# matter-labs/era-zkevm_test_harness

Measured on AMD Instinct MI355X. Metric: base-layer circuits/sec (2^20 rows); full-block synth wall-time 1/8 GPU, higher is better.
Workload: dtype u64 (Goldilocks, p = 2^64 - 2^32 + 1)

## Files before the change

### era_zkevm_test_harness_amd/csrc/gl64.cuh

```cuda
#pragma once
#include <hip/hip_runtime.h>
#include <stdint.h>

namespace gl {

typedef uint64_t u64;
typedef uint32_t u32;

constexpr u64 P = 0xFFFFFFFF00000001ULL;
constexpr u64 EPS = 0xFFFFFFFFULL;

#define GL_HD __host__ __device__ __forceinline__

GL_HD u64 canon(u64 x) { return x >= P ? x - P : x; }

GL_HD u64 add(u64 a, u64 b) {
#if defined(__HIP_DEVICE_COMPILE__)
    unsigned long long s, t;
    const bool c = __builtin_uaddll_overflow(a, b, &s);
    const bool c2 = __builtin_uaddll_overflow(s, c ? EPS : 0, &t);
    return t + (c2 ? EPS : 0);
#else
    u64 s = a + b;
    u64 c = s < a ? EPS : 0;
    u64 t = s + c;
    u64 c2 = t < s ? EPS : 0;
    return t + c2;
#endif
}

GL_HD u64 add_canon(u64 a, u64 c) {
#if defined(__HIP_DEVICE_COMPILE__)
    unsigned long long s;
    const bool w = __builtin_uaddll_overflow(a, c, &s);
    u32 f = w ? 1u : 0u;
    u64 r, dead;
    asm("v_mad_u64_u32 %0, %1, %2, -1, %3" : "=v"(r), "=s"(dead) : "v"(f), "v"((u64)s));
    return r;
#else
    u64 s = a + c;
    return s < a ? s + EPS : s;
#endif
}

GL_HD u64 sub(u64 a, u64 b) {
#if defined(__HIP_DEVICE_COMPILE__)
    unsigned long long d, t;
    const bool br = __builtin_usubll_overflow(a, b, &d);
    const bool br2 = __builtin_usubll_overflow(d, br ? EPS : 0, &t);
    return t - (br2 ? EPS : 0);
#else
    u64 d = a - b;
    u64 br = a < b ? EPS : 0;
    u64 t = d - br;
    u64 br2 = t > d ? EPS : 0;
    return t - br2;
#endif
}

GL_HD u64 neg(u64 a) { return sub(0, a); }

GL_HD u64 reduce128(u64 lo, u64 hi) {
    u64 hh = hi >> 32, hl = hi & EPS;
#if defined(__HIP_DEVICE_COMPILE__)
    unsigned long long t0, r;
    const bool borrow = __builtin_usubll_overflow(lo, hh, &t0);
    t0 -= borrow ? EPS : 0;
    const u64 t1 = (hl << 32) - hl;
    const bool carry = __builtin_uaddll_overflow(t0, t1, &r);
    r += carry ? EPS : 0;
    return r;
#else
    u64 t0 = lo - hh;
    if (lo < hh) t0 -= EPS;
    u64 t1 = hl * EPS;
    u64 r = t0 + t1;
    if (r < t1) r += EPS;
    return r;
#endif
}

#if defined(__HIPCC__)
__device__ __forceinline__ u64 mul_sched(u64 a, u64 b) {
#if !defined(__HIP_DEVICE_COMPILE__)
    return 0;
#else
    const u32 a0 = (u32)a, a1 = (u32)(a >> 32), b0 = (u32)b, b1 = (u32)(b >> 32);
    const u32 zero = 0;
    u64 p, q, h;
    u32 cm;
    asm("v_mad_u64_u32 %0, s[100:101], %4, %6, 0\n\t"
        "v_mad_u64_u32 %1, s[100:101], %4, %7, 0\n\t"
        "v_mad_u64_u32 %2, s[100:101], %5, %7, 0\n\t"
        "v_mad_u64_u32 %1, vcc, %5, %6, %1\n\t"
        "v_addc_co_u32 %3, vcc, 0, %8, vcc"
        : "=&v"(p), "=&v"(q), "=&v"(h), "=&v"(cm)
        : "v"(a0), "v"(a1), "v"(b0), "v"(b1), "v"(zero)
        : "vcc", "s100", "s101");
    const u32 p0 = (u32)p, p1 = (u32)(p >> 32), q0 = (u32)q, q1 = (u32)(q >> 32), h0 = (u32)h, h1 = (u32)(h >> 32);
    u32 r0, r1, w1, g0, g1, m, t0, t1;
    asm("v_add_co_u32 %2, vcc, %8, %10\n\t"
        "v_addc_co_u32 %3, vcc, %12, %11, vcc\n\t"
        "v_addc_co_u32 %4, vcc, %13, %14, vcc\n\t"
        "v_sub_co_u32 %0, vcc, %9, %4\n\t"
        "v_subbrev_co_u32 %1, vcc, 0, %2, vcc\n\t"
        "v_cndmask_b32 %5, 0, -1, vcc\n\t"
        "v_sub_co_u32 %0, vcc, %0, %5\n\t"
        "v_subbrev_co_u32 %1, vcc, 0, %1, vcc\n\t"
        "v_sub_co_u32 %6, vcc, 0, %3\n\t"
        "v_subbrev_co_u32 %7, vcc, 0, %3, vcc\n\t"
        "v_add_co_u32 %0, vcc, %0, %6\n\t"
        "v_addc_co_u32 %1, vcc, %1, %7, vcc\n\t"
        "v_cndmask_b32 %5, 0, -1, vcc\n\t"
        "v_add_co_u32 %0, vcc, %0, %5\n\t"
        "v_addc_co_u32 %1, vcc, 0, %1, vcc"
        : "=&v"(r0), "=&v"(r1), "=&v"(w1), "=&v"(g0), "=&v"(g1), "=&v"(m), "=&v"(t0), "=&v"(t1)
        : "v"(p1), "v"(p0), "v"(q0), "v"(q1), "v"(h0), "v"(h1), "v"(cm)
        : "vcc");
    return ((u64)r1 << 32) | r0;
#endif
}
#endif

#if defined(__HIPCC__)
__device__ __forceinline__ u64 mul_cyc(u64 a, u64 b) {
#if !defined(__HIP_DEVICE_COMPILE__)
    return 0;
#else
    const u32 a0 = (u32)a, a1 = (u32)(a >> 32), b0 = (u32)b, b1 = (u32)(b >> 32);
    u64 p, q, h, x, cm, c1, cw, cw2, bw, b1f, dead;
    asm("v_mad_u64_u32 %0, %1, %2, %3, 0" : "=v"(p), "=s"(dead) : "v"(a0), "v"(b0));
    asm("v_mad_u64_u32 %0, %1, %2, %3, 0" : "=v"(q), "=s"(dead) : "v"(a0), "v"(b1));
    asm("v_mad_u64_u32 %0, %1, %2, %3, 0" : "=v"(h), "=s"(dead) : "v"(a1), "v"(b1));
    asm("v_mad_u64_u32 %0, %1, %2, %3, %4" : "=v"(q), "=s"(cm) : "v"(a1), "v"(b0), "v"(q));
    const u32 p0 = (u32)p, p1 = (u32)(p >> 32), q0 = (u32)q, q1 = (u32)(q >> 32), h0 = (u32)h, h1 = (u32)(h >> 32);
    u32 w1, w2, w3, y0, y1, dlo, dhi;
    asm("v_add_co_u32_e64 %0, %1, %2, %3" : "=v"(w1), "=s"(cw) : "v"(p1), "v"(q0));
    asm("v_addc_co_u32_e64 %0, %1, %2, %3, %4" : "=v"(w2), "=s"(cw2) : "v"(h0), "v"(q1), "s"(cw));
    asm("v_addc_co_u32_e64 %0, %1, %2, 0, %3" : "=v"(w3), "=s"(dead) : "v"(h1), "s"(cw2));
    const u64 lo = ((u64)w1 << 32) | p0;
    asm("v_mad_u64_u32 %0, %1, %2, -1, %3" : "=v"(x), "=s"(c1) : "v"(w2), "v"(lo));
    const u32 x0 = (u32)x, x1 = (u32)(x >> 32);
    asm("v_subb_co_u32_e64 %0, %1, %2, %3, %4" : "=v"(y0), "=s"(bw) : "v"(x0), "v"(w3), "s"(cm));
    asm("v_subbrev_co_u32_e64 %0, %1, 0, %2, %3" : "=v"(y1), "=s"(b1f) : "v"(x1), "s"(bw));
    const u64 mp = c1 & ~b1f, mn = b1f & ~c1;
    asm("v_cndmask_b32_e64 %0, 0, -1, %1" : "=v"(dhi) : "s"(mn));
    asm("v_cndmask_b32_e64 %0, 0, 1, %1" : "=v"(dlo) : "s"(mn));
    asm("v_cndmask_b32_e64 %0, %1, -1, %2" : "=v"(dlo) : "v"(dlo), "s"(mp));
    u64 d = ((u64)dhi << 32) | dlo;
    asm("" : "+v"(d));
    return (((u64)y1 << 32) | y0) + d;
#endif
}
#endif

GL_HD u64 mul_lat(u64 a, u64 b) {
#if defined(__HIP_DEVICE_COMPILE__) && defined(GL_MUL_SCHEDULED_EVERYWHERE)
    return mul_sched(a, b);
#else
#if defined(__HIP_DEVICE_COMPILE__)
    const u32 a0 = (u32)a, a1 = (u32)(a >> 32), b0 = (u32)b, b1 = (u32)(b >> 32);
    const u64 t = (u64)a0 * b0;
    const u64 t1 = (u64)a0 * b1 + (t >> 32);
    const u64 t2 = (u64)a1 * b0 + (u32)t1;
    u64 lo = (t2 << 32) | (u32)t;
    u64 hi = (u64)a1 * b1 + (t1 >> 32) + (t2 >> 32);
#else
    unsigned __int128 w = (unsigned __int128)a * b;
    u64 lo = (u64)w, hi = (u64)(w >> 64);
#endif
    return reduce128(lo, hi);
#endif
}

GL_HD u64 mul(u64 a, u64 b) {
#if defined(__HIP_DEVICE_COMPILE__) && !defined(GL_MUL_COMPILER_FORM)
    return mul_cyc(a, b);
#else
    return mul_lat(a, b);
#endif
}

GL_HD u64 sqr(u64 a) { return mul(a, a); }

GL_HD u64 mul_add(u64 a, u64 b, u64 c) { return add(mul(a, b), c); }

GL_HD u64 pow7(u64 x) {
    u64 x2 = sqr(x);
    u64 x3 = mul(x2, x);
    u64 x4 = sqr(x2);
    return mul(x3, x4);
}
GL_HD u64 pow7_lat(u64 x) {
    u64 x2 = mul_lat(x, x);
    u64 x3 = mul_lat(x2, x);
    u64 x4 = mul_lat(x2, x2);
    return mul_lat(x3, x4);
}

GL_HD u64 mul_pow2(u64 x, u32 s) {
    u64 lo = x << s;
    u64 hi = s ? (x >> (64 - s)) : 0;
    u64 t1 = (hi << 32) - hi;
    u64 r = lo + t1;
    if (r < t1) r += EPS;
    return r;
}

GL_HD u64 mul_small(u64 x, u32 k) {
    u64 l = (x & EPS) * k;
    u64 h = (x >> 32) * k;
    u64 hh = h >> 32, hl = h & EPS;
    u64 r = l + (hl << 32);
    u64 c = r < l ? EPS : 0;
    u64 t = hh * EPS;
    u64 r2 = r + c;
    u64 r3 = r2 + t;
    if (r3 < t) r3 += EPS;
    return r3;
}

GL_HD u64 pow(u64 a, u64 e) {
    u64 r = 1;
    while (e) {
        if (e & 1) r = mul(r, a);
        a = sqr(a);
        e >>= 1;
    }
    return r;
}

GL_HD u64 sqr_n(u64 a, int n) {
    for (int i = 0; i < n; i++) a = sqr(a);
    return a;
}
GL_HD u64 inv(u64 a) {
    const u64 e2 = mul(sqr(a), a);
    const u64 e3 = mul(sqr(e2), a);
    const u64 e6 = mul(sqr_n(e3, 3), e3);
    const u64 e12 = mul(sqr_n(e6, 6), e6);
    const u64 e24 = mul(sqr_n(e12, 12), e12);
    const u64 e30 = mul(sqr_n(e24, 6), e6);
    const u64 e31 = mul(sqr(e30), a);
    const u64 e32 = mul(sqr(e31), a);
    return mul(sqr_n(e31, 33), e32);
}

}
```

### era_zkevm_test_harness_amd/csrc/poseidon2.cuh

```cuda
#pragma once
#include "gl64.cuh"
#include "../../include/zkw_poseidon2_params.h"

namespace p2 {
using gl::u32;
using gl::u64;

static __constant__ u64 c_rc[P2_TOTAL_ROUNDS * P2_WIDTH] = P2_ROUND_CONSTANTS_INIT;
static __constant__ u32 c_shift[P2_WIDTH] = P2_INTERNAL_DIAG_SHIFTS_INIT;

__host__ __device__ __forceinline__ u64 rc_at(int i) {
#if defined(__HIP_DEVICE_COMPILE__)
    return c_rc[i];
#else
    return P2_ROUND_CONSTANTS[i];
#endif
}
__host__ __device__ __forceinline__ u32 shift_at(int i) {
#if defined(__HIP_DEVICE_COMPILE__)
    return c_shift[i];
#else
    return P2_INTERNAL_DIAG_SHIFTS[i];
#endif
}

struct Wide {
    u64 lo;
    u32 hi;
};
GL_HD Wide wide(u64 x) { Wide r; r.lo = x; r.hi = 0; return r; }
GL_HD Wide wadd(Wide a, Wide b) {
    Wide r;
    r.lo = a.lo + b.lo;
    r.hi = a.hi + b.hi + (r.lo < a.lo ? 1u : 0u);
    return r;
}
GL_HD Wide wshl(Wide a, u32 s) {
    Wide r;
    r.lo = a.lo << s;
    r.hi = (a.hi << s) | (u32)(a.lo >> (64 - s));
    return r;
}
GL_HD u64 wreduce(Wide a) {
    u64 t = ((u64)a.hi << 32) - a.hi;
    u64 r = a.lo + t;
    u64 c = r < t ? gl::EPS : 0;
    return r + c;
}

GL_HD void m4w(const u64 x[4], Wide t[4]) {
    Wide t0 = wadd(wide(x[0]), wide(x[1])), t1 = wadd(wide(x[2]), wide(x[3]));
    Wide t2 = wadd(wshl(wide(x[1]), 1), t1), t3 = wadd(wshl(wide(x[3]), 1), t0);
    Wide t4 = wadd(wshl(t1, 2), t3), t5 = wadd(wshl(t0, 2), t2);
    t[0] = wadd(t3, t5); t[1] = t5; t[2] = wadd(t2, t4); t[3] = t4;
}

#if defined(__HIP_DEVICE_COMPILE__)
__device__ __forceinline__ u64 mad_acc(u32 a, u32 k, u64 acc) {
    u64 r, dead;
    asm("v_mad_u64_u32 %0, %1, %2, %3, %4" : "=v"(r), "=s"(dead) : "v"(a), "s"(k), "v"(acc));
    return r;
}
__device__ __forceinline__ u64 mad_acc1(u32 a, u64 acc) {
    u64 r, dead;
    asm("v_mad_u64_u32 %0, %1, %2, 1, %3" : "=v"(r), "=s"(dead) : "v"(a), "v"(acc));
    return r;
}
__device__ __forceinline__ u64 mad_acc2(u32 a, u64 acc) {
    u64 r, dead;
    asm("v_mad_u64_u32 %0, %1, %2, 2, %3" : "=v"(r), "=s"(dead) : "v"(a), "v"(acc));
    return r;
}
__device__ __forceinline__ u64 wp_reduce(u64 L, u64 H) {
    const u32 l0 = (u32)L, l1 = (u32)(L >> 32), h0 = (u32)H, h1 = (u32)(H >> 32);
    u32 n1, k, f;
    u64 c, c2, dead, r;
    asm("v_add_co_u32_e64 %0, %1, %2, %3" : "=v"(n1), "=s"(c) : "v"(l1), "v"(h0));
    asm("v_addc_co_u32_e64 %0, %1, %2, 0, %3" : "=v"(k), "=s"(dead) : "v"(h1), "s"(c));
    const u64 x = ((u64)n1 << 32) | l0;
    asm("v_mad_u64_u32 %0, %1, %2, -1, %3" : "=v"(r), "=s"(c2) : "v"(k), "v"(x));
    asm("v_cndmask_b32_e64 %0, 0, 1, %1" : "=v"(f) : "s"(c2));
    asm("v_mad_u64_u32 %0, %1, %2, -1, %3" : "=v"(r), "=s"(dead) : "v"(f), "v"(r));
    return r;
}
__device__ __forceinline__ void m4_plane(u32 a0, u32 a1, u32 a2, u32 a3, u64 y[4]) {
    const u64 t0 = mad_acc1(a0, (u64)a1), t1 = mad_acc1(a2, (u64)a3);
    const u64 t2 = mad_acc2(a1, t1), t3 = mad_acc2(a3, t0);
    const u64 t4 = (t1 << 2) + t3, t5 = (t0 << 2) + t2;
    y[0] = t3 + t5; y[1] = t5; y[2] = t2 + t4; y[3] = t4;
}
#endif

GL_HD void external(u64 s[12]) {
#if defined(__HIP_DEVICE_COMPILE__) && !defined(P2_LINEAR_WIDE)
    u64 L[12], H[12];
#pragma unroll
    for (int b = 0; b < 3; b++) {
        m4_plane((u32)s[4 * b], (u32)s[4 * b + 1], (u32)s[4 * b + 2], (u32)s[4 * b + 3], L + 4 * b);
        m4_plane((u32)(s[4 * b] >> 32), (u32)(s[4 * b + 1] >> 32), (u32)(s[4 * b + 2] >> 32), (u32)(s[4 * b + 3] >> 32), H + 4 * b);
    }
#pragma unroll
    for (int i = 0; i < 4; i++) {
        const u64 cl = L[i] + L[4 + i] + L[8 + i], ch = H[i] + H[4 + i] + H[8 + i];
#pragma unroll
        for (int b = 0; b < 3; b++) s[4 * b + i] = wp_reduce(L[4 * b + i] + cl, H[4 * b + i] + ch);
    }
#else
    Wide t[12];
    m4w(s, t); m4w(s + 4, t + 4); m4w(s + 8, t + 8);
#pragma unroll
    for (int i = 0; i < 4; i++) {
        Wide col = wadd(wadd(t[i], t[4 + i]), t[8 + i]);
        s[i] = wreduce(wadd(t[i], col)); s[4 + i] = wreduce(wadd(t[4 + i], col)); s[8 + i] = wreduce(wadd(t[8 + i], col));
    }
#endif
}

GL_HD void internal(u64 s[12]) {
    constexpr u32 SH[12] = P2_INTERNAL_DIAG_SHIFTS_INIT;
#if defined(__HIP_DEVICE_COMPILE__) && !defined(P2_LINEAR_WIDE)
    u64 sl = (u64)(u32)s[0], sh = s[0] >> 32;
#pragma unroll
    for (int i = 1; i < 12; i++) { sl = mad_acc1((u32)s[i], sl); sh = mad_acc1((u32)(s[i] >> 32), sh); }
#pragma unroll
    for (int i = 0; i < 12; i++) {
        const u64 l = SH[i] ? mad_acc((u32)s[i], 1u << SH[i], sl) : mad_acc1((u32)s[i], sl);
        const u64 h = SH[i] ? mad_acc((u32)(s[i] >> 32), 1u << SH[i], sh) : mad_acc1((u32)(s[i] >> 32), sh);
        s[i] = wp_reduce(l, h);
    }
#else
    Wide sum = wide(s[0]);
#pragma unroll
    for (int i = 1; i < 12; i++) sum = wadd(sum, wide(s[i]));
#pragma unroll
    for (int i = 0; i < 12; i++) s[i] = wreduce(wadd(SH[i] ? wshl(wide(s[i]), SH[i]) : wide(s[i]), sum));
#endif
}

#ifndef P2_SBOX_GROUP
#define P2_SBOX_GROUP 3
#endif
template <bool LAT = false>
GL_HD void full_round(u64 s[12], int r) {
#pragma unroll
    for (int i = 0; i < 12; i++) {
        s[i] = LAT ? gl::pow7_lat(gl::add_canon(s[i], rc_at(12 * r + i))) : gl::pow7(gl::add_canon(s[i], rc_at(12 * r + i)));
#if defined(__HIP_DEVICE_COMPILE__)
        if (!LAT && (i + 1) % P2_SBOX_GROUP == 0) __builtin_amdgcn_sched_barrier(0);
#endif
    }
    external(s);
}

template <bool LAT = false>
GL_HD void partial_round(u64 s[12], int r) {
    s[0] = LAT ? gl::pow7_lat(gl::add_canon(s[0], rc_at(12 * r))) : gl::pow7(gl::add_canon(s[0], rc_at(12 * r)));
    internal(s);
}

template <bool LAT = false>
GL_HD void permute(u64 s[12]) {
    external(s);
    int r = 0;
    for (int k = 0; k < P2_HALF_FULL_ROUNDS; k++, r++) full_round<LAT>(s, r);
    for (int k = 0; k < P2_PARTIAL_ROUNDS; k++, r++) partial_round<LAT>(s, r);
    for (int k = 0; k < P2_HALF_FULL_ROUNDS; k++, r++) full_round<LAT>(s, r);
}
GL_HD void permute_lat(u64 s[12]) { permute<true>(s); }

#if defined(__HIPCC__)
template <int CTRL>
__device__ __forceinline__ u32 dpp32(u32 v) {
    return (u32)__builtin_amdgcn_update_dpp((int)0, (int)v, CTRL, 0xF, 0xF, false);
}
template <int CTRL>
__device__ __forceinline__ u64 dpp64(u64 v) {
    u32 lo = dpp32<CTRL>((u32)v), hi = dpp32<CTRL>((u32)(v >> 32));
    return ((u64)hi << 32) | lo;
}
constexpr int QP_ROT1 = 1 | (2 << 2) | (3 << 4) | (0 << 6);
constexpr int QP_ROT2 = 2 | (3 << 2) | (0 << 4) | (1 << 6);
constexpr int QP_ROT3 = 3 | (0 << 2) | (1 << 4) | (2 << 6);
constexpr int QP_SWAP1 = 1 | (0 << 2) | (3 << 4) | (2 << 6);
constexpr int QP_BCAST0 = 0;
constexpr int ROW_ROR4 = 0x124, ROW_ROR8 = 0x128, ROW_ROR12 = 0x12C;

template <int CTRL>
__device__ __forceinline__ Wide wdpp(Wide a) {
    Wide r;
    r.lo = dpp64<CTRL>(a.lo);
    r.hi = dpp32<CTRL>(a.hi);
    return r;
}
__device__ __forceinline__ u64 add_rc_sched(u64 x, u64 c) {
    u32 r0, r1, m;
    asm("v_add_co_u32 %0, vcc, %3, %5\n\t"
        "v_addc_co_u32 %1, vcc, %4, %6, vcc\n\t"
        "v_cndmask_b32 %2, 0, -1, vcc\n\t"
        "v_add_co_u32 %0, vcc, %0, %2\n\t"
        "v_addc_co_u32 %1, vcc, 0, %1, vcc"
        : "=&v"(r0), "=&v"(r1), "=&v"(m)
        : "v"((u32)x), "v"((u32)(x >> 32)), "v"((u32)c), "v"((u32)(c >> 32))
        : "vcc");
    return ((u64)r1 << 32) | r0;
}
__device__ __forceinline__ u64 pow7_sched(u64 x) {
    const u64 x2 = gl::mul_sched(x, x), x3 = gl::mul_sched(x2, x), x4 = gl::mul_sched(x2, x2);
    return gl::mul_sched(x3, x4);
}

struct Coop {
    u64 rc_full[2 * P2_HALF_FULL_ROUNDS];
    u32 ka, kb, kd;
    u32 shift;
    u32 rsh, hi_mask;
    bool active;
    bool first;
    bool second;

    __device__ __forceinline__ void init(int g) {
        active = g < 12;
        first = g == 0;
        second = g == 1;
#pragma unroll
        for (int k = 0; k < 2 * P2_HALF_FULL_ROUNDS; k++) {
            int round = k < P2_HALF_FULL_ROUNDS ? k : k + P2_PARTIAL_ROUNDS;
            rc_full[k] = active ? c_rc[12 * round + g] : 0;
        }
        bool even = (g & 1) == 0;
        ka = even ? 5u : 6u;
        kb = even ? 7u : 1u;
        kd = even ? 3u : 4u;
        shift = active ? c_shift[g] : 0;
        rsh = (32u - shift) & 31u;
        hi_mask = shift ? 0xffffffffu : 0u;
    }

    __device__ __forceinline__ u64 external(u64 x) const {
        u64 a = x, b = dpp64<QP_ROT1>(x), c = dpp64<QP_ROT2>(x), d = dpp64<QP_ROT3>(x);
        u64 L = (a & gl::EPS) * ka + (b & gl::EPS) * kb + (c & gl::EPS) + (d & gl::EPS) * kd;
        u64 H = (a >> 32) * ka + (b >> 32) * kb + (c >> 32) + (d >> 32) * kd;
        u32 r0, r1, t0, t1, t2, u0, u1, u2, e0, e1, e2;
        asm volatile(
            "v_add_co_u32 %3, vcc, %11, %13\n\t"
            "v_addc_co_u32 %4, vcc, 0, %14, vcc\n\t"
            "s_nop 0\n\t"
            "v_add_co_u32_dpp %5, vcc, %12, %12 row_ror:8 row_mask:0xf bank_mask:0xf\n\t"
            "v_addc_co_u32_dpp %6, vcc, %3, %3, vcc row_ror:8 row_mask:0xf bank_mask:0xf\n\t"
            "v_addc_co_u32_dpp %7, vcc, %4, %4, vcc row_ror:8 row_mask:0xf bank_mask:0xf\n\t"
            "v_add_co_u32_dpp %5, vcc, %5, %5 row_ror:4 row_mask:0xf bank_mask:0xf\n\t"
            "v_addc_co_u32_dpp %6, vcc, %6, %6, vcc row_ror:4 row_mask:0xf bank_mask:0xf\n\t"
            "v_addc_co_u32_dpp %7, vcc, %7, %7, vcc row_ror:4 row_mask:0xf bank_mask:0xf\n\t"
            "v_add_co_u32 %0, vcc, %12, %5\n\t"
            "v_addc_co_u32 %1, vcc, %3, %6, vcc\n\t"
            "v_addc_co_u32 %2, vcc, %4, %7, vcc\n\t"
            "v_sub_co_u32 %8, vcc, 0, %2\n\t"
            "v_subbrev_co_u32 %9, vcc, 0, %2, vcc\n\t"
            "v_add_co_u32 %0, vcc, %0, %8\n\t"
            "v_addc_co_u32 %1, vcc, %1, %9, vcc\n\t"
            "v_cndmask_b32 %10, 0, -1, vcc\n\t"
            "v_add_co_u32 %0, vcc, %0, %10\n\t"
            "v_addc_co_u32 %1, vcc, 0, %1, vcc"
            : "=&v"(r0), "=&v"(r1), "=&v"(t0), "=&v"(t1), "=&v"(t2), "=&v"(u0), "=&v"(u1), "=&v"(u2), "=&v"(e0), "=&v"(e1), "=&v"(e2)
            : "v"((u32)(L >> 32)), "v"((u32)L), "v"((u32)H), "v"((u32)(H >> 32))
            : "vcc");
        const u64 y = ((u64)r1 << 32) | r0;
        return active ? y : 0;
    }

    __device__ __forceinline__ u64 internal(u64 x) const {
        const u32 x0 = (u32)x, x1 = (u32)(x >> 32);
        u32 s0, s1, s2;
        const u32 zero = 0;
        asm volatile(
            "s_nop 1\n\t"
            "v_add_co_u32_dpp %0, vcc, %3, %3 row_ror:8 row_mask:0xf bank_mask:0xf\n\t"
            "v_addc_co_u32_dpp %1, vcc, %4, %4, vcc row_ror:8 row_mask:0xf bank_mask:0xf\n\t"
            "v_addc_co_u32 %2, vcc, 0, %5, vcc\n\t"
            "v_add_co_u32_dpp %0, vcc, %0, %0 row_ror:4 row_mask:0xf bank_mask:0xf\n\t"
            "v_addc_co_u32_dpp %1, vcc, %1, %1, vcc row_ror:4 row_mask:0xf bank_mask:0xf\n\t"
            "v_addc_co_u32_dpp %2, vcc, %2, %2, vcc row_ror:4 row_mask:0xf bank_mask:0xf\n\t"
            "v_add_co_u32_dpp %0, vcc, %0, %0 quad_perm:[2,3,0,1] row_mask:0xf bank_mask:0xf\n\t"
            "v_addc_co_u32_dpp %1, vcc, %1, %1, vcc quad_perm:[2,3,0,1] row_mask:0xf bank_mask:0xf\n\t"
            "v_addc_co_u32_dpp %2, vcc, %2, %2, vcc quad_perm:[2,3,0,1] row_mask:0xf bank_mask:0xf\n\t"
            "v_add_co_u32_dpp %0, vcc, %0, %0 quad_perm:[1,0,3,2] row_mask:0xf bank_mask:0xf\n\t"
            "v_addc_co_u32_dpp %1, vcc, %1, %1, vcc quad_perm:[1,0,3,2] row_mask:0xf bank_mask:0xf\n\t"
            "v_addc_co_u32_dpp %2, vcc, %2, %2, vcc quad_perm:[1,0,3,2] row_mask:0xf bank_mask:0xf"
            : "=&v"(s0), "=&v"(s1), "=&v"(s2)
            : "v"(x0), "v"(x1), "v"(zero)
            : "vcc");
        const u64 mlo = x << shift;
        const u32 m2 = (x1 >> rsh) & hi_mask;
        u32 r0, r1;
        u32 t0, t1, t2, t3;
        asm volatile(
            "v_add_co_u32 %0, vcc, %6, %9\n\t"
            "v_addc_co_u32 %1, vcc, %7, %10, vcc\n\t"
            "v_addc_co_u32 %2, vcc, %8, %11, vcc\n\t"
            "v_sub_co_u32 %3, vcc, 0, %2\n\t"
            "v_subbrev_co_u32 %4, vcc, 0, %2, vcc\n\t"
            "v_add_co_u32 %0, vcc, %0, %3\n\t"
            "v_addc_co_u32 %1, vcc, %1, %4, vcc\n\t"
            "v_cndmask_b32 %5, 0, -1, vcc\n\t"
            "v_add_co_u32 %0, vcc, %0, %5\n\t"
            "v_addc_co_u32 %1, vcc, 0, %1, vcc"
            : "=&v"(r0), "=&v"(r1), "=&v"(t0), "=&v"(t1), "=&v"(t2), "=&v"(t3)
            : "v"((u32)mlo), "v"((u32)(mlo >> 32)), "v"(m2), "v"(s0), "v"(s1), "v"(s2)
            : "vcc");
        const u64 y = ((u64)r1 << 32) | r0;
        return active ? y : 0;
    }

    __device__ __forceinline__ u64 permute(u64 x) const {
        x = external(x);
#pragma unroll
        for (int k = 0; k < P2_HALF_FULL_ROUNDS; k++) x = external(pow7_sched(add_rc_sched(x, rc_full[k])));
        for (int k = 0; k < P2_PARTIAL_ROUNDS; k++) {
            u64 rc = c_rc[12 * (P2_HALF_FULL_ROUNDS + k)];
            u64 sx = pow7_pair(add_rc_sched(x, rc));
            x = internal(first ? sx : x);
        }
#pragma unroll
        for (int k = 0; k < P2_HALF_FULL_ROUNDS; k++)
            x = external(pow7_sched(add_rc_sched(x, rc_full[P2_HALF_FULL_ROUNDS + k])));
        return x;
    }

    __device__ __forceinline__ u64 pow7_pair(u64 t) const {
        const u64 t0 = dpp64<QP_BCAST0>(t);
        const u64 x2 = gl::mul_sched(t0, t0);
        const u64 b = second ? x2 : t0;
        const u64 y = gl::mul_sched(x2, b);
        return gl::mul_sched(y, dpp64<QP_SWAP1>(y));
    }
};

template <class Put>
__device__ __forceinline__ u64 coop_flattened(const Coop& co, u64 x, u32 g, Put&& put) {
    if (co.active) put(g, gl::canon(x));
    x = co.external(x);
#pragma unroll
    for (int k = 0; k < P2_HALF_FULL_ROUNDS; k++) {
        x = co.external(pow7_sched(add_rc_sched(x, co.rc_full[k])));
        if (co.active) put(12 * (k + 1) + g, gl::canon(x));
    }
    for (int k = 0; k < P2_PARTIAL_ROUNDS; k++) {
        const u64 rc = c_rc[12 * (P2_HALF_FULL_ROUNDS + k)];
        const u64 sx = co.pow7_pair(add_rc_sched(x, rc));
        if (co.first) put(12 * (P2_HALF_FULL_ROUNDS + 1) + k, gl::canon(sx));
        x = co.internal(co.first ? sx : x);
    }
#pragma unroll
    for (int k = 0; k < P2_HALF_FULL_ROUNDS; k++) {
        x = co.external(pow7_sched(add_rc_sched(x, co.rc_full[P2_HALF_FULL_ROUNDS + k])));
        if (co.active) put(12 * (P2_HALF_FULL_ROUNDS + 1) + P2_PARTIAL_ROUNDS + 12 * k + g, gl::canon(x));
    }
    return gl::canon(x);
}


#if defined(P2_Q4_PARTIAL_SCHED)
#define Q4_PARTIAL_MUL gl::mul_sched
#else
#define Q4_PARTIAL_MUL gl::mul_lat
#endif
#if defined(P2_Q4_FULL_CYC)
#define Q4_FULL_POW7 gl::pow7
#else
#define Q4_FULL_POW7 gl::pow7_lat
#endif
template <int CTRL>
__device__ __forceinline__ u32 qdpp32(u32 v) {
    return (u32)__builtin_amdgcn_update_dpp((int)0, (int)v, CTRL, 0xF, 0xF, true);
}
template <int CTRL>
__device__ __forceinline__ u64 qdpp64(u64 v) {
    return ((u64)qdpp32<CTRL>((u32)(v >> 32)) << 32) | qdpp32<CTRL>((u32)v);
}

struct Coop4 {
    u64 rc_full[2 * P2_HALF_FULL_ROUNDS][3];
    u32 ka, kb, kd;
    u32 pw[3];
    bool first;
    bool second;

    __device__ __forceinline__ void init(int j) {
        first = j == 0;
        second = j == 1;
#pragma unroll
        for (int k = 0; k < 2 * P2_HALF_FULL_ROUNDS; k++) {
            int round = k < P2_HALF_FULL_ROUNDS ? k : k + P2_PARTIAL_ROUNDS;
#pragma unroll
            for (int c = 0; c < 3; c++) rc_full[k][c] = c_rc[12 * round + 4 * c + j];
        }
        bool even = (j & 1) == 0;
        ka = even ? 5u : 6u;
        kb = even ? 7u : 1u;
        kd = even ? 3u : 4u;
#pragma unroll
        for (int c = 0; c < 3; c++) pw[c] = 1u << c_shift[4 * c + j];
    }

#if defined(__HIP_DEVICE_COMPILE__)
    static __device__ __forceinline__ u64 mad_v(u32 a, u32 k, u64 acc) {
        u64 r, dead;
        asm("v_mad_u64_u32 %0, %1, %2, %3, %4" : "=v"(r), "=s"(dead) : "v"(a), "v"(k), "v"(acc));
        return r;
    }
    template <bool SC = false>
    static __device__ __forceinline__ u64 add_rc(u64 x, u32 c0, u32 c1);
#endif

    __device__ __forceinline__ u64 m4_plane(u32 a) const {
        const u32 b = qdpp32<QP_ROT1>(a), c = qdpp32<QP_ROT2>(a), d = qdpp32<QP_ROT3>(a);
#if defined(__HIP_DEVICE_COMPILE__)
        return mad_v(d, kd, mad_v(b, kb, mad_v(a, ka, (u64)c)));
#else
        return (u64)a * ka + (u64)b * kb + c + (u64)d * kd;
#endif
    }

    __device__ __forceinline__ void external(u64 x[3]) const {
#if defined(__HIP_DEVICE_COMPILE__)
        u64 L[3], H[3];
#pragma unroll
        for (int c = 0; c < 3; c++) { L[c] = m4_plane((u32)x[c]); H[c] = m4_plane((u32)(x[c] >> 32)); }
        const u64 cl = L[0] + L[1] + L[2], ch = H[0] + H[1] + H[2];
#pragma unroll
        for (int c = 0; c < 3; c++) x[c] = wp_reduce(L[c] + cl, H[c] + ch);
#endif
    }

    __device__ __forceinline__ void internal(u64 x[3]) const {
#if defined(__HIP_DEVICE_COMPILE__)
        const u64 pl = mad_acc1((u32)x[0], mad_acc1((u32)x[1], (u64)(u32)x[2]));
        const u64 ph = mad_acc1((u32)(x[0] >> 32), mad_acc1((u32)(x[1] >> 32), x[2] >> 32));
        u32 l0, l1, h0, h1;
        asm volatile(
            "s_nop 1\n\t"
            "v_add_co_u32_dpp %0, vcc, %4, %4 quad_perm:[2,3,0,1] row_mask:0xf bank_mask:0xf\n\t"
            "v_addc_co_u32_dpp %1, vcc, %5, %5, vcc quad_perm:[2,3,0,1] row_mask:0xf bank_mask:0xf\n\t"
            "v_add_co_u32_dpp %2, vcc, %6, %6 quad_perm:[2,3,0,1] row_mask:0xf bank_mask:0xf\n\t"
            "v_addc_co_u32_dpp %3, vcc, %7, %7, vcc quad_perm:[2,3,0,1] row_mask:0xf bank_mask:0xf\n\t"
            "v_add_co_u32_dpp %0, vcc, %0, %0 quad_perm:[1,0,3,2] row_mask:0xf bank_mask:0xf\n\t"
            "v_addc_co_u32_dpp %1, vcc, %1, %1, vcc quad_perm:[1,0,3,2] row_mask:0xf bank_mask:0xf\n\t"
            "v_add_co_u32_dpp %2, vcc, %2, %2 quad_perm:[1,0,3,2] row_mask:0xf bank_mask:0xf\n\t"
            "v_addc_co_u32_dpp %3, vcc, %3, %3, vcc quad_perm:[1,0,3,2] row_mask:0xf bank_mask:0xf"
            : "=&v"(l0), "=&v"(l1), "=&v"(h0), "=&v"(h1)
            : "v"((u32)pl), "v"((u32)(pl >> 32)), "v"((u32)ph), "v"((u32)(ph >> 32))
            : "vcc");
        const u64 sl = ((u64)l1 << 32) | l0, sh = ((u64)h1 << 32) | h0;
#pragma unroll
        for (int c = 0; c < 3; c++) x[c] = wp_reduce(mad_v((u32)x[c], pw[c], sl), mad_v((u32)(x[c] >> 32), pw[c], sh));
#endif
    }

    __device__ __forceinline__ void permute(u64 x[3]) const {
#if defined(__HIP_DEVICE_COMPILE__)
        constexpr u64 RC[P2_TOTAL_ROUNDS * P2_WIDTH] = P2_ROUND_CONSTANTS_INIT;
        external(x);
#pragma unroll
        for (int k = 0; k < P2_HALF_FULL_ROUNDS; k++) {
#pragma unroll
            for (int c = 0; c < 3; c++) x[c] = Q4_FULL_POW7(add_rc(x[c], (u32)rc_full[k][c], (u32)(rc_full[k][c] >> 32)));
            external(x);
        }
#pragma unroll
        for (int k = 0; k < P2_PARTIAL_ROUNDS; k++) {
            constexpr int R0 = 12 * P2_HALF_FULL_ROUNDS;
            const u64 rc = RC[R0 + 12 * k];
            const u64 t0 = qdpp64<QP_BCAST0>(add_rc<true>(x[0], (u32)rc, (u32)(rc >> 32)));
            const u64 x2 = Q4_PARTIAL_MUL(t0, t0);
            const u64 y = Q4_PARTIAL_MUL(x2, second ? x2 : t0);
            const u64 sx = Q4_PARTIAL_MUL(y, qdpp64<QP_SWAP1>(y));
            x[0] = first ? sx : x[0];
            internal(x);
        }
#pragma unroll
        for (int k = 0; k < P2_HALF_FULL_ROUNDS; k++) {
#pragma unroll
            for (int c = 0; c < 3; c++)
                x[c] = Q4_FULL_POW7(add_rc(x[c], (u32)rc_full[P2_HALF_FULL_ROUNDS + k][c], (u32)(rc_full[P2_HALF_FULL_ROUNDS + k][c] >> 32)));
            external(x);
        }
#endif
    }
};
#if defined(__HIP_DEVICE_COMPILE__)
#define P2_Q4_ADD_RC(C0)                                                             \
    asm("v_add_co_u32 %0, vcc, %3, %5\n\t"                                          \
        "v_addc_co_u32 %1, vcc, %4, %6, vcc\n\t"                                    \
        "v_subb_co_u32 %2, vcc, %0, %0, vcc"           \
        : "=&v"(r0), "=&v"(r1), "=&v"(m)                                              \
        : C0(c0), "v"(c1), "v"((u32)x), "v"((u32)(x >> 32))                           \
        : "vcc")
template <bool SC>
__device__ __forceinline__ u64 Coop4::add_rc(u64 x, u32 c0, u32 c1) {
    u32 r0, r1, m;
    if constexpr (SC) P2_Q4_ADD_RC("s"); else P2_Q4_ADD_RC("v");
    return mad_acc1(m, ((u64)r1 << 32) | r0);
}
#undef P2_Q4_ADD_RC
#endif

struct Coop2 {
    u64 rc_full[2 * P2_HALF_FULL_ROUNDS][6];
    u32 shift[6];
    bool first;

    __device__ __forceinline__ void init(int j) {
        first = j == 0;
#pragma unroll
        for (int k = 0; k < 2 * P2_HALF_FULL_ROUNDS; k++) {
            const int round = k < P2_HALF_FULL_ROUNDS ? k : k + P2_PARTIAL_ROUNDS;
#pragma unroll
            for (int c = 0; c < 3; c++) {
                rc_full[k][2 * c] = c_rc[12 * round + 4 * c + 2 * j];
                rc_full[k][2 * c + 1] = c_rc[12 * round + 4 * c + 2 * j + 1];
            }
        }
#pragma unroll
        for (int c = 0; c < 3; c++) {
            shift[2 * c] = c_shift[4 * c + 2 * j];
            shift[2 * c + 1] = c_shift[4 * c + 2 * j + 1];
        }
    }

    __device__ __forceinline__ void external(u64 x[6]) const {
        Wide A[3], B[3];
#pragma unroll
        for (int c = 0; c < 3; c++) {
            const Wide own = wadd(wide(x[2 * c]), wide(x[2 * c + 1]));
            const Wide oth = wdpp<QP_SWAP1>(own);
            const u64 p1 = dpp64<QP_SWAP1>(x[2 * c + 1]);
            B[c] = wadd(wadd(wshl(own, 2), wshl(wide(x[2 * c + 1]), 1)), oth);
            A[c] = wadd(wadd(B[c], wshl(wide(p1), 1)), own);
        }
        const Wide colA = wadd(wadd(A[0], A[1]), A[2]), colB = wadd(wadd(B[0], B[1]), B[2]);
#pragma unroll
        for (int c = 0; c < 3; c++) {
            x[2 * c] = wreduce(wadd(A[c], colA));
            x[2 * c + 1] = wreduce(wadd(B[c], colB));
        }
    }

    __device__ __forceinline__ void internal(u64 x[6]) const {
        Wide s = wide(x[0]);
#pragma unroll
        for (int i = 1; i < 6; i++) s = wadd(s, wide(x[i]));
        s = wadd(s, wdpp<QP_SWAP1>(s));
#pragma unroll
        for (int i = 0; i < 6; i++) {
            Wide m;
            m.lo = x[i] << shift[i];
            m.hi = (u32)((x[i] >> 1) >> (63 - shift[i]));
            x[i] = wreduce(wadd(m, s));
        }
    }

    __device__ __forceinline__ void permute(u64 x[6]) const {
        external(x);
#pragma unroll
        for (int k = 0; k < P2_HALF_FULL_ROUNDS; k++) {
#pragma unroll
            for (int i = 0; i < 6; i++) x[i] = gl::pow7_lat(gl::add(x[i], rc_full[k][i]));
            external(x);
        }
        for (int k = 0; k < P2_PARTIAL_ROUNDS; k++) {
            const u64 rc = c_rc[12 * (P2_HALF_FULL_ROUNDS + k)];
            const u64 sx = gl::pow7_lat(gl::add(x[0], rc));
            x[0] = first ? sx : x[0];
            internal(x);
        }
#pragma unroll
        for (int k = 0; k < P2_HALF_FULL_ROUNDS; k++) {
#pragma unroll
            for (int i = 0; i < 6; i++) x[i] = gl::pow7_lat(gl::add(x[i], rc_full[P2_HALF_FULL_ROUNDS + k][i]));
            external(x);
        }
    }
};
#endif

}
```

Baseline: 3049.

## Hand-schedule Goldilocks mul/sqr/reduce in asm for Coop4 Poseidon2 rounds

Adds hand-written inline-asm Goldilocks multiply, square (three partial products plus a shift instead of four) and a shared reduction, and uses them for the full-round pow7 and the partial-round S-box in the cooperative 4-lane Poseidon2 permutation. It also rewrites the external and internal linear layers as batched v_mad_u64_u32 sequences with a three-way fused Goldilocks reduction, replacing the per-element mad_v and wp_reduce calls. The goal is fewer VALU instructions and shorter dependency chains in the hash inner loop. In exchange it removes the compile-time selectable multiply variants, and because the asm blocks reuse vcc heavily they may limit compiler scheduling or hide subtle carry bugs.

```diff
diff --git a/era_zkevm_test_harness_amd/csrc/gl64.cuh b/era_zkevm_test_harness_amd/csrc/gl64.cuh
--- a/era_zkevm_test_harness_amd/csrc/gl64.cuh
+++ b/era_zkevm_test_harness_amd/csrc/gl64.cuh
@@ -120,6 +120,69 @@
     return ((u64)r1 << 32) | r0;
 #endif
 }
+
+__device__ __forceinline__ u64 lone_reduce(u64 p, u64 q, u64 h, u32 cm) {
+#if !defined(__HIP_DEVICE_COMPILE__)
+    return 0;
+#else
+    u32 y0, y1, w2, w3, m;
+    asm("v_add_co_u32 %1, vcc, %5, %7\n\t"
+        "v_addc_co_u32 %2, vcc, %9, %8, vcc\n\t"
+        "v_addc_co_u32 %3, vcc, %10, %11, vcc\n\t"
+        "v_sub_co_u32 %0, vcc, %6, %3\n\t"
+        "v_subbrev_co_u32 %1, vcc, 0, %1, vcc\n\t"
+        "v_subb_co_u32 %4, vcc, %3, %3, vcc\n\t"
+        "v_sub_co_u32 %0, vcc, %0, %4\n\t"
+        "v_subbrev_co_u32 %1, vcc, 0, %1, vcc"
+        : "=&v"(y0), "=&v"(y1), "=&v"(w2), "=&v"(w3), "=&v"(m)
+        : "v"((u32)(p >> 32)), "v"((u32)p), "v"((u32)q), "v"((u32)(q >> 32)), "v"((u32)h), "v"((u32)(h >> 32)), "v"(cm)
+        : "vcc");
+    u64 r = ((u64)y1 << 32) | y0;
+    asm("v_mad_u64_u32 %0, vcc, %2, -1, %0\n\t"
+        "v_subb_co_u32 %1, vcc, %2, %2, vcc\n\t"
+        "v_mad_u64_u32 %0, vcc, %1, 1, %0"
+        : "+v"(r), "=&v"(m)
+        : "v"(w2)
+        : "vcc");
+    return r;
+#endif
+}
+__device__ __forceinline__ u64 mul_lone(u64 a, u64 b) {
+#if !defined(__HIP_DEVICE_COMPILE__)
+    return 0;
+#else
+    u64 p, q, h;
+    u32 cm;
+    asm("v_mad_u64_u32 %0, vcc, %4, %6, 0\n\t"
+        "v_mad_u64_u32 %1, vcc, %4, %7, 0\n\t"
+        "v_mad_u64_u32 %2, vcc, %5, %7, 0\n\t"
+        "v_mad_u64_u32 %1, vcc, %5, %6, %1\n\t"
+        "v_addc_co_u32 %3, vcc, 0, %8, vcc"
+        : "=&v"(p), "=&v"(q), "=&v"(h), "=&v"(cm)
+        : "v"((u32)a), "v"((u32)(a >> 32)), "v"((u32)b), "v"((u32)(b >> 32)), "v"(0u)
+        : "vcc");
+    return lone_reduce(p, q, h, cm);
+#endif
+}
+__device__ __forceinline__ u64 sqr_lone(u64 a) {
+#if !defined(__HIP_DEVICE_COMPILE__)
+    return 0;
+#else
+    u64 p, q, q2, h;
+    asm("v_mad_u64_u32 %0, vcc, %4, %4, 0\n\t"
+        "v_mad_u64_u32 %1, vcc, %4, %5, 0\n\t"
+        "v_mad_u64_u32 %3, vcc, %5, %5, 0\n\t"
+        "v_lshl_add_u64 %2, %1, 1, 0"
+        : "=&v"(p), "=&v"(q), "=&v"(q2), "=&v"(h)
+        : "v"((u32)a), "v"((u32)(a >> 32))
+        : "vcc");
+    return lone_reduce(p, q2, h, (u32)(q >> 63));
+#endif
+}
+__device__ __forceinline__ u64 pow7_lone(u64 x) {
+    const u64 x2 = sqr_lone(x), x3 = mul_lone(x2, x), x4 = sqr_lone(x2);
+    return mul_lone(x3, x4);
+}
 #endif
 
 #if defined(__HIPCC__)
diff --git a/era_zkevm_test_harness_amd/csrc/poseidon2.cuh b/era_zkevm_test_harness_amd/csrc/poseidon2.cuh
--- a/era_zkevm_test_harness_amd/csrc/poseidon2.cuh
+++ b/era_zkevm_test_harness_amd/csrc/poseidon2.cuh
@@ -359,16 +359,6 @@
 }
 
 
-#if defined(P2_Q4_PARTIAL_SCHED)
-#define Q4_PARTIAL_MUL gl::mul_sched
-#else
-#define Q4_PARTIAL_MUL gl::mul_lat
-#endif
-#if defined(P2_Q4_FULL_CYC)
-#define Q4_FULL_POW7 gl::pow7
-#else
-#define Q4_FULL_POW7 gl::pow7_lat
-#endif
 template <int CTRL>
 __device__ __forceinline__ u32 qdpp32(u32 v) {
     return (u32)__builtin_amdgcn_update_dpp((int)0, (int)v, CTRL, 0xF, 0xF, true);
@@ -403,21 +393,52 @@
     }
 
 #if defined(__HIP_DEVICE_COMPILE__)
-    static __device__ __forceinline__ u64 mad_v(u32 a, u32 k, u64 acc) {
-        u64 r, dead;
-        asm("v_mad_u64_u32 %0, %1, %2, %3, %4" : "=v"(r), "=s"(dead) : "v"(a), "v"(k), "v"(acc));
-        return r;
+    static __device__ __forceinline__ void wp_reduce3(const u64 L[3], const u64 H[3], u64 x[3]) {
+        u32 n0 = (u32)(L[0] >> 32), n1 = (u32)(L[1] >> 32), n2 = (u32)(L[2] >> 32), k0, k1, k2, m;
+        asm("v_add_co_u32 %0, vcc, %0, %6\n\t"
+            "v_addc_co_u32 %3, vcc, 0, %7, vcc\n\t"
+            "v_add_co_u32 %1, vcc, %1, %8\n\t"
+            "v_addc_co_u32 %4, vcc, 0, %9, vcc\n\t"
+            "v_add_co_u32 %2, vcc, %2, %10\n\t"
+            "v_addc_co_u32 %5, vcc, 0, %11, vcc"
+            : "+v"(n0), "+v"(n1), "+v"(n2), "=&v"(k0), "=&v"(k1), "=&v"(k2)
+            : "v"((u32)H[0]), "v"((u32)(H[0] >> 32)), "v"((u32)H[1]), "v"((u32)(H[1] >> 32)), "v"((u32)H[2]), "v"((u32)(H[2] >> 32))
+            : "vcc");
+        u64 r0 = ((u64)n0 << 32) | (u32)L[0], r1 = ((u64)n1 << 32) | (u32)L[1], r2 = ((u64)n2 << 32) | (u32)L[2];
+        asm("v_mad_u64_u32 %0, vcc, %4, -1, %0\n\t"
+            "v_subb_co_u32 %3, vcc, %4, %4, vcc\n\t"
+            "v_mad_u64_u32 %0, vcc, %3, 1, %0\n\t"
+            "v_mad_u64_u32 %1, vcc, %5, -1, %1\n\t"
+            "v_subb_co_u32 %3, vcc, %5, %5, vcc\n\t"
+            "v_mad_u64_u32 %1, vcc, %3, 1, %1\n\t"
+            "v_mad_u64_u32 %2, vcc, %6, -1, %2\n\t"
+            "v_subb_co_u32 %3, vcc, %6, %6, vcc\n\t"
+            "v_mad_u64_u32 %2, vcc, %3, 1, %2"
+            : "+v"(r0), "+v"(r1), "+v"(r2), "=&v"(m)
+            : "v"(k0), "v"(k1), "v"(k2)
+            : "vcc");
+        x[0] = r0; x[1] = r1; x[2] = r2;
     }
     template <bool SC = false>
     static __device__ __forceinline__ u64 add_rc(u64 x, u32 c0, u32 c1);
 #endif
 
-    __device__ __forceinline__ u64 m4_plane(u32 a) const {
+    __device__ __forceinline__ void m4_planes(u64 x, u64& L, u64& H) const {
+#if defined(__HIP_DEVICE_COMPILE__)
+        const u32 a = (u32)x, e = (u32)(x >> 32);
         const u32 b = qdpp32<QP_ROT1>(a), c = qdpp32<QP_ROT2>(a), d = qdpp32<QP_ROT3>(a);
-#if defined(__HIP_DEVICE_COMPILE__)
-        return mad_v(d, kd, mad_v(b, kb, mad_v(a, ka, (u64)c)));
+        const u32 f = qdpp32<QP_ROT1>(e), g = qdpp32<QP_ROT2>(e), h = qdpp32<QP_ROT3>(e);
+        asm("v_mad_u64_u32 %0, vcc, %2, %10, %8\n\t"
+            "v_mad_u64_u32 %1, vcc, %5, %10, %9\n\t"
+            "v_mad_u64_u32 %0, vcc, %3, %11, %0\n\t"
+            "v_mad_u64_u32 %1, vcc, %6, %11, %1\n\t"
+            "v_mad_u64_u32 %0, vcc, %4, %12, %0\n\t"
+            "v_mad_u64_u32 %1, vcc, %7, %12, %1"
+            : "=&v"(L), "=&v"(H)
+            : "v"(a), "v"(b), "v"(d), "v"(e), "v"(f), "v"(h), "v"((u64)c), "v"((u64)g), "v"(ka), "v"(kb), "v"(kd)
+            : "vcc");
 #else
-        return (u64)a * ka + (u64)b * kb + c + (u64)d * kd;
+        L = H = 0;
 #endif
     }
 
@@ -425,17 +446,24 @@
 #if defined(__HIP_DEVICE_COMPILE__)
         u64 L[3], H[3];
 #pragma unroll
-        for (int c = 0; c < 3; c++) { L[c] = m4_plane((u32)x[c]); H[c] = m4_plane((u32)(x[c] >> 32)); }
+        for (int c = 0; c < 3; c++) m4_planes(x[c], L[c], H[c]);
         const u64 cl = L[0] + L[1] + L[2], ch = H[0] + H[1] + H[2];
 #pragma unroll
-        for (int c = 0; c < 3; c++) x[c] = wp_reduce(L[c] + cl, H[c] + ch);
+        for (int c = 0; c < 3; c++) { L[c] += cl; H[c] += ch; }
+        wp_reduce3(L, H, x);
 #endif
     }
 
     __device__ __forceinline__ void internal(u64 x[3]) const {
 #if defined(__HIP_DEVICE_COMPILE__)
-        const u64 pl = mad_acc1((u32)x[0], mad_acc1((u32)x[1], (u64)(u32)x[2]));
-        const u64 ph = mad_acc1((u32)(x[0] >> 32), mad_acc1((u32)(x[1] >> 32), x[2] >> 32));
+        u64 pl, ph;
+        asm("v_mad_u64_u32 %0, vcc, %2, 1, %6\n\t"
+            "v_mad_u64_u32 %1, vcc, %3, 1, %7\n\t"
+            "v_mad_u64_u32 %0, vcc, %4, 1, %0\n\t"
+            "v_mad_u64_u32 %1, vcc, %5, 1, %1"
+            : "=&v"(pl), "=&v"(ph)
+            : "v"((u32)x[1]), "v"((u32)(x[1] >> 32)), "v"((u32)x[0]), "v"((u32)(x[0] >> 32)), "v"((u64)(u32)x[2]), "v"(x[2] >> 32)
+            : "vcc");
         u32 l0, l1, h0, h1;
         asm volatile(
             "s_nop 1\n\t"
@@ -451,8 +479,18 @@
             : "v"((u32)pl), "v"((u32)(pl >> 32)), "v"((u32)ph), "v"((u32)(ph >> 32))
             : "vcc");
         const u64 sl = ((u64)l1 << 32) | l0, sh = ((u64)h1 << 32) | h0;
-#pragma unroll
-        for (int c = 0; c < 3; c++) x[c] = wp_reduce(mad_v((u32)x[c], pw[c], sl), mad_v((u32)(x[c] >> 32), pw[c], sh));
+        u64 L[3], H[3];
+        asm("v_mad_u64_u32 %0, vcc, %6, %12, %15\n\t"
+            "v_mad_u64_u32 %1, vcc, %7, %12, %16\n\t"
+            "v_mad_u64_u32 %2, vcc, %8, %13, %15\n\t"
+            "v_mad_u64_u32 %3, vcc, %9, %13, %16\n\t"
+            "v_mad_u64_u32 %4, vcc, %10, %14, %15\n\t"
+            "v_mad_u64_u32 %5, vcc, %11, %14, %16"
+            : "=&v"(L[0]), "=&v"(H[0]), "=&v"(L[1]), "=&v"(H[1]), "=&v"(L[2]), "=&v"(H[2])
+            : "v"((u32)x[0]), "v"((u32)(x[0] >> 32)), "v"((u32)x[1]), "v"((u32)(x[1] >> 32)), "v"((u32)x[2]), "v"((u32)(x[2] >> 32)),
+              "v"(pw[0]), "v"(pw[1]), "v"(pw[2]), "v"(sl), "v"(sh)
+            : "vcc");
+        wp_reduce3(L, H, x);
 #endif
     }
 
@@ -463,7 +501,7 @@
 #pragma unroll
         for (int k = 0; k < P2_HALF_FULL_ROUNDS; k++) {
 #pragma unroll
-            for (int c = 0; c < 3; c++) x[c] = Q4_FULL_POW7(add_rc(x[c], (u32)rc_full[k][c], (u32)(rc_full[k][c] >> 32)));
+            for (int c = 0; c < 3; c++) x[c] = gl::pow7_lone(add_rc(x[c], (u32)rc_full[k][c], (u32)(rc_full[k][c] >> 32)));
             external(x);
         }
 #pragma unroll
@@ -471,9 +509,9 @@
             constexpr int R0 = 12 * P2_HALF_FULL_ROUNDS;
             const u64 rc = RC[R0 + 12 * k];
             const u64 t0 = qdpp64<QP_BCAST0>(add_rc<true>(x[0], (u32)rc, (u32)(rc >> 32)));
-            const u64 x2 = Q4_PARTIAL_MUL(t0, t0);
-            const u64 y = Q4_PARTIAL_MUL(x2, second ? x2 : t0);
-            const u64 sx = Q4_PARTIAL_MUL(y, qdpp64<QP_SWAP1>(y));
+            const u64 x2 = gl::sqr_lone(t0);
+            const u64 y = gl::mul_lone(x2, second ? x2 : t0);
+            const u64 sx = gl::mul_lone(y, qdpp64<QP_SWAP1>(y));
             x[0] = first ? sx : x[0];
             internal(x);
         }
@@ -481,7 +519,7 @@
         for (int k = 0; k < P2_HALF_FULL_ROUNDS; k++) {
 #pragma unroll
             for (int c = 0; c < 3; c++)
-                x[c] = Q4_FULL_POW7(add_rc(x[c], (u32)rc_full[P2_HALF_FULL_ROUNDS + k][c], (u32)(rc_full[P2_HALF_FULL_ROUNDS + k][c] >> 32)));
+                x[c] = gl::pow7_lone(add_rc(x[c], (u32)rc_full[P2_HALF_FULL_ROUNDS + k][c], (u32)(rc_full[P2_HALF_FULL_ROUNDS + k][c] >> 32)));
             external(x);
         }
 #endif
```

After: 3059 (median of 3 runs). Within noise of the previous version (+0.3%).
